# r9y9/deepvoice3_pytorch

Hardware: AMD Instinct MI355X
Metric: mel-frames/sec/node (train step, deepvoice3_ljspeech) (higher is better)
Workload: dtype f16x3

## Files before the change

### deepvoice3_pytorch_amd/csrc/attention.hip

```cpp
#include "common.h"

namespace {

__global__ __launch_bounds__(256) void attn_softmax_kernel(const dv3_softmax_desc p) {
  const int lane = threadIdx.x & 63;
  const int64_t row = (int64_t)blockIdx.x * 4 + (threadIdx.x >> 6);
  if (row >= (int64_t)p.B * p.Tq) return;
  const int b = (int)(row / p.Tq);
  const int Tk = p.Tk;
  float* s = p.s + row * Tk;
  int lo = 0, hi = Tk;
  if (p.key_len) hi = min(hi, p.key_len[b]);
  if (p.last_attended) {
    const int la = p.last_attended[0];
    const int wlo = la - p.win_back, whi = la + p.win_ahead;
    if (wlo > 0) lo = max(lo, wlo);
    if (whi < Tk) hi = min(hi, whi);
  }
  float mx = -INFINITY;
  for (int n = lo + lane; n < hi; n += 64) mx = fmaxf(mx, s[n]);
  mx = dv3_wave_max(mx);
  float sum = 0.f;
  for (int n = lo + lane; n < hi; n += 64) sum += expf(s[n] - mx);
  sum = dv3_wave_sum(sum);
// ... 128 lines not shown
    for (int r = 0; r < 16; ++r) acc[r] = 0.f;
    auto fetch3 = [&](int n0, float (&a)[16], float (&bv)[16]) __attribute__((always_inline)) {
#pragma unroll
      for (int i = 0; i < 16; ++i) {
        const int n = n0 + 2 * i + lhi;
        const int nn = min(n, Tk - 1);
        const float av = vtb[(int64_t)nn * E + e];
        bv[i] = sc[l31 * ld + nn];
        a[i] = n < Tk ? av : 0.f;
      }
    };
    float a0[16], b0[16], a1[16], b1[16];
    fetch3(0, a0, b0);
    for (int n0 = 0; n0 < Tk; n0 += 64) {
      if (n0 + 32 < Tk) fetch3(n0 + 32, a1, b1);
#pragma unroll
      for (int i = 0; i < 16; ++i) acc = __builtin_amdgcn_mfma_f32_32x32x2f32(a0[i], b0[i], acc, 0, 0, 0);
      if (n0 + 32 >= Tk) break;
      if (n0 + 64 < Tk) fetch3(n0 + 64, a0, b0);
#pragma unroll
      for (int i = 0; i < 16; ++i) acc = __builtin_amdgcn_mfma_f32_32x32x2f32(a1[i], b1[i], acc, 0, 0, 0);
    }
    const int t = t0 + l31;
    if (t < Tq) {
#pragma unroll
      for (int r = 0; r < 16; ++r) {
        const int ec = et * 32 + (r & 3) + 8 * (r >> 2) + 4 * lhi;
        if (ec < E) p.ctx[((int64_t)b * E + ec) * Tq + t] = acc[r];
      }
    }
  }
}

__global__ __launch_bounds__(64) void attn_argmax_kernel(const float* __restrict__ p, int Tk,
                                                         int32_t* __restrict__ out) {
  const int lane = threadIdx.x;
  float best = -INFINITY;
  int bi = 0x7fffffff;
  for (int n = lane; n < Tk; n += 64) {
    const float v = p[n];
    if (v > best) { best = v; bi = n; }
  }
#pragma unroll
  for (int off = 32; off > 0; off >>= 1) {
    const float ov = __shfl_xor(best, off, 64);
    const int oi = __shfl_xor(bi, off, 64);
    if (ov > best || (ov == best && oi < bi)) { best = ov; bi = oi; }
  }
  if (lane == 0) out[0] = bi;
}

}

extern "C" int dv3_attn_softmax_f32(const dv3_softmax_desc* d, void* stream) {
  DV3_REQUIRE(d && d->s && d->B > 0 && d->Tq > 0 && d->Tk > 0, "attn_softmax: bad args");
  if (d->mask) DV3_REQUIRE(d->pd && d->mask_rs * 32 >= d->Tk, "attn_softmax: mask needs pd and a wide enough row stride");
  const int64_t rows = (int64_t)d->B * d->Tq;
  hipLaunchKernelGGL(attn_softmax_kernel, dim3((unsigned)dv3_cdiv64(rows, 4)), dim3(256), 0,
                     (hipStream_t)stream, *d);
  return dv3_check_launch("attn_softmax_f32");
}

extern "C" int dv3_attn_softmax_bwd_f32(const dv3_softmax_bwd_desc* d, void* stream) {
  DV3_REQUIRE(d && d->p && d->ds && (d->dpd || d->dp_direct), "attn_softmax_bwd: bad args");
  DV3_REQUIRE(d->B > 0 && d->Tq > 0 && d->Tk > 0, "attn_softmax_bwd: bad dims");
  const int64_t rows = (int64_t)d->B * d->Tq;
  hipLaunchKernelGGL(attn_softmax_bwd_kernel, dim3((unsigned)dv3_cdiv64(rows, 4)), dim3(256), 0,
                     (hipStream_t)stream, *d);
  return dv3_check_launch("attn_softmax_bwd_f32");
}

extern "C" int dv3_attn_fwd_f32(const dv3_attn_fwd_desc* d, void* stream) {
  DV3_REQUIRE(d && d->q && d->k && d->vT && d->ctx && d->P && d->pd, "attn_fwd: null pointer");
  DV3_REQUIRE(d->B > 0 && d->E > 0 && d->Tq > 0 && d->Tk > 0 && d->B <= 65535, "attn_fwd: bad dims");
  if (d->mask) DV3_REQUIRE(d->mask_rs * 32 >= d->Tk, "attn_fwd: mask row stride too small");
  const size_t lds = (size_t)32 * (d->Tk + 1) * sizeof(float);
  DV3_REQUIRE(lds <= 64 * 1024, "attn_fwd: Tk = %d too long for the fused kernel (use the unfused path)", d->Tk);
  hipLaunchKernelGGL(attn_fwd_kernel, dim3(dv3_cdiv(d->Tq, 32), d->B), dim3(256), lds, (hipStream_t)stream, *d);
  return dv3_check_launch("attn_fwd");
}

extern "C" int dv3_attn_argmax_i32(const float* p_row, int32_t Tk, int32_t* out, void* stream) {
  DV3_REQUIRE(p_row && out && Tk > 0, "attn_argmax: bad args");
  hipLaunchKernelGGL(attn_argmax_kernel, dim3(1), dim3(64), 0, (hipStream_t)stream, p_row, Tk, out);
  return dv3_check_launch("attn_argmax_i32");
}
```

### deepvoice3_pytorch_amd/csrc/loss.hip

```cpp
#include "common.h"

namespace {

constexpr int kLossBlock = 256;

struct spec_loss_args : dv3_spec_loss_desc {
  float* dpre; float* bias_part;
};

__device__ __forceinline__ void block_reduce4(float v[4], float* out , float* extra = nullptr) {
  __shared__ float red[4][4];
#pragma unroll
  for (int k = 0; k < 4; ++k) v[k] = dv3_wave_sum(v[k]);
  const int w = threadIdx.x >> 6;
  if ((threadIdx.x & 63) == 0) {
#pragma unroll
    for (int k = 0; k < 4; ++k) red[w][k] = v[k];
  }
  __syncthreads();
  if (threadIdx.x < 4) {
    const float sum = red[0][threadIdx.x] + red[1][threadIdx.x] + red[2][threadIdx.x] + red[3][threadIdx.x];
    out[threadIdx.x] = sum;
    if (extra && threadIdx.x == 1) extra[0] = sum;
  }
// ... 198 lines not shown
        }
      }
      if (sums)
        for (int dl = dw; dl < nd; dl += 4) ys[tl * 65 + dl] = 0.f;
    }
    if (HEAD && tt_ == t_tiles - 1) {
      for (int tz = Tr + tl; tz < p.T; tz += 64) {
        int64_t ih = b * p.yh_bs + tz + (int64_t)(d0 + dw) * p.yh_ds;
        for (int dl = dw; dl < nd; dl += 4, ih += ihs) {
          p.dpre[ih] = 0.f;
          if (p.dyh) p.dyh[ih] = 0.f;
        }
      }
    }
    if (sums) {
      __syncthreads();
      const int bin = tid >> 2, part = tid & 3;
      float v[16];
#pragma unroll
      for (int i = 0; i < 16; ++i) v[i] = ys[(part * 16 + i) * 65 + bin];
#pragma unroll
      for (int w = 1; w < 16; w <<= 1)
#pragma unroll
        for (int i = 0; i < 16; i += 2 * w) v[i] += v[i + w];
      float s = v[0];
      s += __shfl_xor(s, 1, 4);
      s += __shfl_xor(s, 2, 4);
      if (part == 0 && bin < nd) p.bias_part[(int64_t)(d0 + bin) * n_part + (int64_t)b * t_tiles + tt_] = s;
    }
  }
  block_reduce4(acc, p.scratch + (int64_t)blockIdx.x * 4);
}

__global__ __launch_bounds__(256) void spec_loss_tail_zero_kernel(const dv3_spec_loss_desc p) {
  const int64_t n = (int64_t)p.B * p.r * p.D;
  const int64_t i = (int64_t)blockIdx.x * 256 + threadIdx.x;
  if (i >= n) return;
  const int dd = (int)(i % p.D);
  const int64_t bt = i / p.D;
  const int t = p.T - p.r + (int)(bt % p.r);
  const int b = (int)(bt / p.r);
  p.dyh[b * p.yh_bs + t * p.yh_ts + dd * p.yh_ds] = 0.f;
}

__global__ __launch_bounds__(256) void spec_loss_finish_kernel(const dv3_spec_loss_desc p,
                                                               int n_blocks) {
  float acc[4] = {0.f, 0.f, 0.f, 0.f};
  for (int i = threadIdx.x; i < n_blocks; i += 256)
#pragma unroll
    for (int k = 0; k < 4; ++k) acc[k] += p.scratch[(int64_t)i * 4 + k];
  __shared__ float fin[4];
  block_reduce4(acc, fin);
  __syncthreads();
  if (threadIdx.x == 0) {
    const bool use_mask = p.w_masked > 0.f && p.lengths;
    const float msum = use_mask ? spec_mask_sum(p) : 1.f;
    const float n = (float)((int64_t)p.B * (spec_t_valid(p) - p.r) * p.D);
    const float wm = use_mask ? p.w_masked : 0.f;
    const float l1 = wm * (use_mask ? fin[1] / msum : 0.f) + (1.f - wm) * fin[0] / n;
    const float bd = p.w_bd > 0.f ? wm * (use_mask ? fin[3] / msum : 0.f) + (1.f - wm) * fin[2] / n : 0.f;
    p.out4[0] = l1;
    p.out4[1] = bd;
    p.out4[2] = (1.f - p.w_bd) * l1 + p.w_bd * bd;
    p.out4[3] = msum;
  }
}

__device__ __forceinline__ float guided_w(int nk, int t, int N, int T, double inv2g2) {
  const double dlt = (double)nk / (double)N - (double)t / (double)T;
  return (float)(1.0 - exp(-dlt * dlt * inv2g2));
}

__global__ __launch_bounds__(256) void guided_attn_kernel(const float* __restrict__ attn,
                                                          const int32_t* __restrict__ in_len,
                                                          const int32_t* __restrict__ out_len,
                                                          float* __restrict__ dattn,
                                                          float* __restrict__ scratch, int L, int B,
                                                          int Tq, int Tk, float g, float gscale,
                                                          const int32_t* __restrict__ tq_valid,
                                                          const int32_t* __restrict__ tk_valid) {
  const int64_t per = (int64_t)B * Tq * Tk;
  const int64_t n = tq_valid ? (int64_t)L * B * min(tq_valid[0], Tq) * min(tk_valid[0], Tk) : per * L;
  const float inv_n = 1.0f / (float)n;
// ... 152 lines not shown
}

__global__ __launch_bounds__(256) void items_finish_kernel(const float* __restrict__ scratch, int B, int slices,
                                                           int n_sums, float* __restrict__ out,
                                                           const int32_t* __restrict__ len_a, int sub_a, int cap_a,
                                                           const int32_t* __restrict__ len_b, int cap_b,
                                                           int64_t mult) {
  const int b = blockIdx.x * 256 + threadIdx.x;
  if (b >= B) return;
  float acc[2] = {0.f, 0.f};
  for (int s = 0; s < slices; ++s)
    for (int k = 0; k < n_sums; ++k) acc[k] += scratch[((int64_t)b * slices + s) * 4 + k];
  int64_t cnt = mult * clamp_len(len_a[b] - sub_a, cap_a);
  if (len_b) cnt *= clamp_len(len_b[b], cap_b);
  float* row = out + (int64_t)b * (n_sums + 1);
  for (int k = 0; k < n_sums; ++k) row[k] = acc[k];
  row[n_sums] = (float)cnt;
}

template <class Desc>
inline bool spec_time_fast(const Desc& d) {
  return d.yh_ts == 1 && d.y_ds == 1 && d.yh_ds > 1 && d.y_ts > 1 && (int64_t)d.B * d.yh_bs < (1ll << 40);
}

inline int loss_blocks(int64_t n) {
  int64_t b = dv3_cdiv64(n, (int64_t)kLossBlock * 4);
  if (b < 1) b = 1;
  if (b > 1024) b = 1024;
  return (int)b;
}

}


extern "C" int dv3_spec_loss_scratch_floats(int32_t B, int32_t T, int32_t D) {
  int64_t tiles = (int64_t)B * dv3_cdiv(T, 64) * dv3_cdiv(D, 64);
  if (tiles > 1024) tiles = 1024;
  const int64_t flat = loss_blocks((int64_t)B * T * D);
  return (int)(4 * (tiles > flat ? tiles : flat) + 16);
}

static int spec_loss_launch(const dv3_spec_loss_desc* d, float* dpre, float* bias_part, void* stream) {
  DV3_REQUIRE(d && d->y_hat && d->y && d->out4 && d->scratch, "spec_loss: null pointer");
  DV3_REQUIRE(d->B > 0 && d->D > 0 && d->r >= 0 && d->T > d->r, "spec_loss: bad dims");
  DV3_REQUIRE(d->w_masked <= 0.f || d->lengths, "spec_loss: masked weight needs lengths");
  hipStream_t st = (hipStream_t)stream;
  spec_loss_args a;
  static_cast<dv3_spec_loss_desc&>(a) = *d;
  a.dpre = dpre;
  a.bias_part = bias_part;
  const int64_t n = (int64_t)d->B * (d->T - d->r) * d->D;
  int nb = loss_blocks(n);
  if (spec_time_fast(*d)) {
    const int t_tiles = dv3_cdiv(d->T - d->r, 64), d_tiles = dv3_cdiv(d->D, 64);
    const int64_t nt = (int64_t)d->B * t_tiles * d_tiles;
    nb = (int)(nt < 1024 ? nt : 1024);
    const bool fast_log = dv3_sw(DV3_SW_LOSS_FAST_LOG);
    auto k = dpre ? (fast_log ? spec_loss_tiled_kernel<true, true> : spec_loss_tiled_kernel<false, true>)
                     : (fast_log ? spec_loss_tiled_kernel<true, false> : spec_loss_tiled_kernel<false, false>);
    hipLaunchKernelGGL(k, dim3(nb), dim3(kLossBlock), 0, st, a, t_tiles, d_tiles, (int)nt);
  } else {
    hipLaunchKernelGGL(spec_loss_kernel, dim3(nb), dim3(kLossBlock), 0, st, a);
    if (dpre && bias_part) {
      const int t_tiles = dv3_cdiv(d->T - d->r, 64);
      const int64_t ns = (int64_t)d->B * t_tiles * d->D;
      hipLaunchKernelGGL(spec_head_rowsum_kernel, dim3((unsigned)dv3_cdiv64(ns, 256)), dim3(256), 0, st, a, t_tiles);
    }
  }
  if (d->dyh && !dpre && d->r > 0) {
    const int64_t nt = (int64_t)d->B * d->r * d->D;
    hipLaunchKernelGGL(spec_loss_tail_zero_kernel, dim3((unsigned)dv3_cdiv64(nt, 256)), dim3(256), 0,
                       st, *d);
  }
  hipLaunchKernelGGL(spec_loss_finish_kernel, dim3(1), dim3(256), 0, st, *d, nb);
  return dv3_check_launch("spec_loss_f32");
}

extern "C" int dv3_spec_loss_f32(const dv3_spec_loss_desc* d, void* stream) {
  return spec_loss_launch(d, nullptr, nullptr, stream);
}

extern "C" int dv3_spec_loss_head_f32(const dv3_spec_loss_desc* d, float* dpre, float* bias_part, void* stream) {
  DV3_REQUIRE(dpre, "spec_loss_head: dpre is required");
  return spec_loss_launch(d, dpre, bias_part, stream);
}

extern "C" int dv3_guided_attn_loss_f32(const float* attn, const int32_t* in_len,
                                        const int32_t* out_len, float* dattn, float* out1,
                                        float* scratch, int32_t L, int32_t B, int32_t Tq, int32_t Tk,
                                        float g, float gscale, void* stream) {
  DV3_REQUIRE(attn && in_len && out_len && out1 && scratch, "guided_attn: null pointer");
  DV3_REQUIRE(L > 0 && B > 0 && Tq > 0 && Tk > 0 && g > 0.f, "guided_attn: bad dims");
  hipStream_t st = (hipStream_t)stream;
// ... 50 lines not shown
extern "C" int dv3_bce_loss_head_f32(const float* p, const float* t, float* dp, float* dpre, float* bias_part, float* out1,
                                     float* scratch, int64_t rows, int32_t T, const int32_t* t_valid, float gscale,
                                     void* stream) {
  DV3_REQUIRE(p && t && dpre && out1 && scratch && rows > 0 && T > 0, "bce_loss_head: bad args");
  hipStream_t st = (hipStream_t)stream;
  const int64_t n = rows * T;
  const int nb = loss_blocks(n);
  if (t_valid) {
    hipLaunchKernelGGL(bce_kernel, dim3(nb), dim3(256), 0, st, p, t, dp, scratch, n, gscale, (int)T, t_valid, dpre, bias_part);
    hipLaunchKernelGGL(sum_finish_kernel, dim3(1), dim3(256), 0, st, scratch, nb, 0.f, out1, t_valid, (int)T,
                       (const int32_t*)nullptr, 0, rows);
  } else {
    hipLaunchKernelGGL(bce_kernel, dim3(nb), dim3(256), 0, st, p, t, dp, scratch, n, gscale, 0, (const int32_t*)nullptr, dpre,
                       bias_part);
    hipLaunchKernelGGL(sum_finish_kernel, dim3(1), dim3(256), 0, st, scratch, nb, 1.0f / (float)n, out1,
                       (const int32_t*)nullptr, 0, (const int32_t*)nullptr, 0, (int64_t)0);
  }
  return dv3_check_launch("bce_loss_head_f32");
}

extern "C" int dv3_loss_items_scratch_floats(int32_t B, int32_t T) {
  if (B <= 0 || T <= 0) return 0;
  return (int)((int64_t)4 * B * item_slices(T));
}

extern "C" int dv3_spec_loss_items_f32(const dv3_spec_items_desc* d, void* stream) {
  DV3_REQUIRE(d && d->y_hat && d->y && d->lengths && d->out && d->scratch, "spec_loss_items: null pointer");
  DV3_REQUIRE(d->B > 0 && d->B <= 65535 && d->D > 0 && d->r >= 0 && d->T > 0, "spec_loss_items: bad dims");
  hipStream_t st = (hipStream_t)stream;
  const int Tr = d->T > d->r ? d->T - d->r : 0;
  const int S = Tr > 0 ? item_slices(Tr) : 0;
  if (S > 0) {
    DV3_REQUIRE((int64_t)dv3_cdiv(Tr, S) * d->D < (1ll << 31), "spec_loss_items: slice too large");
    if (spec_time_fast(*d) && dv3_sw(DV3_SW_LOSS_FAST_LOG))
      hipLaunchKernelGGL(spec_items_kernel<true>, dim3(S, d->B), dim3(kLossBlock), 0, st, *d);
    else
      hipLaunchKernelGGL(spec_items_kernel<false>, dim3(S, d->B), dim3(kLossBlock), 0, st, *d);
  }
  hipLaunchKernelGGL(items_finish_kernel, dim3(dv3_cdiv(d->B, 256)), dim3(256), 0, st, (const float*)d->scratch, (int)d->B,
                     S, 2, d->out, d->lengths, (int)d->r, Tr, (const int32_t*)nullptr, 0, (int64_t)d->D);
  return dv3_check_launch("spec_loss_items_f32");
}

extern "C" int dv3_bce_loss_items_f32(const float* p, const float* t, const int32_t* lengths, float* out,
                                      float* scratch, int32_t B, int32_t T, void* stream) {
  DV3_REQUIRE(p && t && lengths && out && scratch, "bce_loss_items: null pointer");
  DV3_REQUIRE(B > 0 && B <= 65535 && T > 0, "bce_loss_items: bad dims");
  hipStream_t st = (hipStream_t)stream;
  const int S = item_slices(T);
  hipLaunchKernelGGL(bce_items_kernel, dim3(S, B), dim3(256), 0, st, p, t, lengths, scratch, (int)T);
  hipLaunchKernelGGL(items_finish_kernel, dim3(dv3_cdiv(B, 256)), dim3(256), 0, st, (const float*)scratch, (int)B, S, 1,
                     out, lengths, 0, (int)T, (const int32_t*)nullptr, 0, (int64_t)1);
  return dv3_check_launch("bce_loss_items_f32");
}

extern "C" int dv3_guided_attn_loss_items_f32(const float* attn, const int32_t* in_len, const int32_t* out_len,
                                              float* out, float* scratch, int32_t L, int32_t B, int32_t Tq,
                                              int32_t Tk, float g, void* stream) {
  DV3_REQUIRE(attn && in_len && out_len && out && scratch, "guided_attn_items: null pointer");
  DV3_REQUIRE(L > 0 && B > 0 && B <= 65535 && Tq > 0 && Tk > 0 && g > 0.f, "guided_attn_items: bad dims");
  hipStream_t st = (hipStream_t)stream;
  const int S = item_slices(Tq);
  DV3_REQUIRE((int64_t)dv3_cdiv(Tq, S) * Tk < (1ll << 31), "guided_attn_items: slice too large");
  hipLaunchKernelGGL(guided_attn_items_kernel, dim3(S, B), dim3(256), 0, st, attn, in_len, out_len, scratch, (int)L,
                     (int)B, (int)Tq, (int)Tk, g);
  hipLaunchKernelGGL(items_finish_kernel, dim3(dv3_cdiv(B, 256)), dim3(256), 0, st, (const float*)scratch, (int)B, S, 1,
                     out, out_len, 0, (int)Tq, in_len, (int)Tk, (int64_t)L);
// ... 3 lines not shown
```

### deepvoice3_pytorch_amd/ops.py

```python
import contextlib
import ctypes
import functools
import math

import torch

from . import _lib
from ._lib import CONSTS, STRUCTS, _env_flag, _env_int, _env_str

EPI_LINEAR = CONSTS["DV3_EPI_LINEAR"]
EPI_RELU = CONSTS["DV3_EPI_RELU"]
EPI_SIGMOID = CONSTS["DV3_EPI_SIGMOID"]
EPI_GLU = CONSTS["DV3_EPI_GLU"]
EPI_HIGHWAY = CONSTS["DV3_EPI_HIGHWAY"]
EPI_DGRAD = CONSTS["DV3_EPI_DGRAD"]
EPI_SOFTSIGN = CONSTS["DV3_EPI_SOFTSIGN"]
STORE_BCT = CONSTS["DV3_STORE_BCT"]
STORE_INTERLEAVE2 = CONSTS["DV3_STORE_INTERLEAVE2"]

_conv_desc = STRUCTS["dv3_conv_desc"]
_wgrad_desc = STRUCTS["dv3_wgrad_desc"]
_wn_desc = STRUCTS["dv3_wn_desc"]
_wn_bwd_desc = STRUCTS["dv3_wn_bwd_desc"]
_gate_bwd_desc = STRUCTS["dv3_gate_bwd_desc"]
# ... 1598 lines not shown
    if (x8 or want8) and not _c8_layer_ok(v, cfg, x8 if want8 is None else bool(want8), x.shape[2]):
        y = ConvLayerFn.apply(from_c8(x, v.shape[1]) if x8 else x, v, g, bias, spk,
                              from_c8(r) if is_c8(r) else r, from_c8(r2) if is_c8(r2) else r2, cfg, packed)
        out8 = x8 if want8 is None else bool(want8)
        return to_c8(y) if out8 else y
    if x8 or want8:
        y = ConvLayerC8Fn.apply(x, v, g, bias, spk, r, r2, cfg, packed)
        if is_c8(y):
            gated = cfg.mode in (EPI_GLU, EPI_HIGHWAY)
            y._dv3_C = v.shape[0] // 2 if gated else v.shape[0]
        return y
    return ConvLayerFn.apply(x, v, g, bias, spk, r, r2, cfg, packed)


def _attn_split(forward=False):
    if forward and _gemm_mode == "f16x3":
        return False
    return _gemm_mode != "f32"


class AttnCoreFn(torch.autograd.Function):
    @staticmethod
    def forward(ctx, q, k, v, key_len, last_attended, cfg):
        q, k, v = _c(_chk(q, "q")), _c(_chk(k, "k")), _c(_chk(v, "v"))
        B, E, Tq = q.shape
        Tk = k.shape[2]
        p_drop, training, win_back, win_ahead, site = cfg
        dev = q.device
        bits, bits_rs, dscale = None, 0, 1.0
        if training and p_drop > 0:
            bits, bits_rs = dropout_bits(B * Tq, Tk, p_drop, dev, site)
            dscale = 1.0 / (1.0 - p_drop)
        if fused_attention and last_attended is None and Tk <= 511 and Tq > 1:
            vT = transpose(v)
            ctxv = torch.empty((B, E, Tq), dtype=torch.float32, device=dev)
            P = torch.empty((B, Tq, Tk), dtype=torch.float32, device=dev)
            pd = torch.empty_like(P)
            d = _attn_fwd_desc()
            d.q, d.k, d.vT, d.key_len = q.data_ptr(), k.data_ptr(), vT.data_ptr(), _ptr(key_len)
            d.mask, d.mask_rs, d.drop_scale = _ptr(bits), bits_rs, dscale
            vs = valid.scale if valid is not None else None
            d.pd_scale = 1.0 if vs is not None else Tk * math.sqrt(1.0 / Tk)
            d.pd_scale_dev = _ptr(vs)
            d.ctx, d.P, d.pd = ctxv.data_ptr(), P.data_ptr(), pd.data_ptr()
            d.B, d.E, d.Tq, d.Tk = B, E, Tq, Tk
            _lib.call("dv3_attn_fwd_f32", ctypes.byref(d), _stream())
            if any(ctx.needs_input_grad[:3]):
                ctx.save_for_backward(q, k, v, P, pd)
                ctx.bits, ctx.bits_rs, ctx.dscale, ctx.pd_scale = bits, bits_rs, dscale, d.pd_scale
                ctx.scale_dev = vs
            return ctxv, P
        S = conv_gemm(k, q, Tq, 0, B=B, Cin=E, Tin=Tk, M=Tq, Tout=Tk, a_bs=E * Tq)
        pd = torch.empty_like(S)
        d = _softmax_desc()
        d.s, d.pd, d.key_len, d.last_attended = S.data_ptr(), pd.data_ptr(), _ptr(key_len), _ptr(last_attended)
        d.mask, d.mask_rs, d.drop_scale = _ptr(bits), bits_rs, dscale
        vs = valid.scale if valid is not None else None
        d.pd_scale = 1.0 if vs is not None else Tk * math.sqrt(1.0 / Tk)
        d.pd_scale_dev = _ptr(vs)
        d.B, d.Tq, d.Tk, d.win_back, d.win_ahead = B, Tq, Tk, win_back, win_ahead
        _lib.call("dv3_attn_softmax_f32", ctypes.byref(d), _stream())
        P = S
        ctxv = wgrad_gemm(v, pd, B=B, M=E, Cin=Tq, T=Tk, Tin=Tk, n_slabs=B,
                          split_bf16=_attn_split(forward=True)).view(B, E, Tq)
        if any(ctx.needs_input_grad[:3]):
            ctx.save_for_backward(q, k, v, P, pd)
            ctx.bits, ctx.bits_rs, ctx.dscale, ctx.pd_scale = bits, bits_rs, dscale, d.pd_scale
            ctx.scale_dev = vs
        return ctxv, P

    @staticmethod
    def backward(ctx, dctx, dP):
# ... 765 lines not shown
```

### include/dv3hip.h

```cpp
#ifndef DV3HIP_H
#define DV3HIP_H

#include <stdint.h>

#ifdef __cplusplus
extern "C" {
#endif

#define DV3_OK 0
#define DV3_EINVAL (-1)
#define DV3_ELAUNCH (-2)

#define DV3_ABI_VERSION 50
int dv3_abi_version(void);
const char* dv3_last_error(void);
int dv3_device_info(int dev, char* name, int name_len, int* n_cu);
int dv3_sizeof(const char* name);
#define DV3_SWITCHES(X) \
  X(2, WGRAD_TILE, 0, 0, 4, "split weight gradient: 0 by rule / 1 128x128 per tap / 2 256x128 per tap / 3 all-taps / 4 two-steps-ahead all-taps") \
  X(3, X3_PINGPONG, 1, 0, 1, "8-wave split tap-GEMM tiles: 0 in-phase / 1 ping-pong main loop") \
  X(4, PLANES_TILE, 0, 0, 9, "planes tap-GEMM tile: 0 by rule, conv_c8pp first / 1 128x128 / 2 128x64 / 9 128x256; any other value: by rule, conv_c8pp kept out") \
  X(12, X3_PP2_MIN_TILES, 128, 0, 2147483647, "256x256 split tap-GEMM serves eligible grids of at least this many tiles (0 never)") \
  X(14, X3_PRIO, 0, 0, 4, "wave priority scheme of the ping-pong split main loop (kernel argument; 0 none)") \
  X(15, WGRAD_PRIO, 0, 0, 2, "wave priority scheme of the all-taps weight gradient (kernel argument; 0 none)") \
  X(17, WGRAD_TAPS2, 1, 0, 1, "all-taps weight gradient by rule: 0 one step ahead / 1 two steps ahead") \
  X(18, X3_WIDE, 1, 0, 1, "16-byte input-gradient epilogue through LDS of the split tap-GEMMs (kernel argument): 0 off / 1 on") \
  X(19, C8PP_MIN_TILES, 128, 0, 2147483647, "conv_c8pp serves eligible grids of at least this many tiles (0 never, 1 always)") \
  X(20, WGRAD_C8_PF2, 1, 0, 1, "register-transposing wgrad_c8: operands fetched 0 one / 1 two steps ahead") \
  X(22, PP2_SK, 1, 0, 3, "stream-K form of the 256x256 split tap-GEMM: 0 never / 1 by rule, forward / 2 whenever a workspace is given / 3 by rule, both directions") \
  X(29, PP2_ORD_U, 81, 0, 81, "LOAD-phase order of the unmasked 256x256 split instantiations: 0, 17 or 81 only") \
  X(30, C8PP_RF, 1, 0, 1, "conv_c8pp LOAD phase: 0 staging first / 1 fragment reads first") \
  X(31, PP2_ORD_M, 81, 0, 81, "LOAD-phase order of the masked 256x256 split instantiations: 0, 17 or 81 only") \
  X(34, C8PP_NW4, 2, 0, 2, "conv_c8pp form: 0 8 waves on 256x256 only / 1 two 4-wave workgroups per CU on 256x128 / 2 by rule") \
  X(35, C8PP_STAGGER, 0, 0, 1024, "conv_c8pp, 4-wave form: start delay (x 64 cycles) of the delayed blocks (kernel argument)") \
  X(36, C8PP_STAGGER_MASK, 1, 0, 2147483647, "conv_c8pp, 4-wave form: blocks with (blockIdx & mask) != 0 are the delayed ones (kernel argument)") \
  X(44, X3_KS, 1, 0, 2, "k-split form of the 128x64 split tile: 0 never / 1 by rule / 2 wherever eligible") \
  X(47, WGRAD_T2_WINDOW, 1, 0, 1, "two-steps-ahead weight gradient, d = 1 / 3: 0 per-tap form / 1 one window for three taps") \
  X(48, WGRAD_T2_IL, 1, 0, 1, "its window forms stage the next tile 0 after / 1 between the MFMAs") \
  X(49, WGRAD_C8_IL, 1, 0, 1, "register-transposing wgrad_c8, three taps: next tile staged 0 after / 1 between the MFMAs") \
  X(50, PP2_FAST_TAIL, 1, 0, 1, "256x256 split tap-GEMM, gated launch: 0 guarded tail everywhere / 1 straight-line tail on interior sub-tiles (kernel argument)") \
  X(51, WN_BWD_VEC4, 1, 0, 1, "weight-norm backward gather: 0 4-byte everywhere / 1 16-byte where aligned") \
  X(52, WGRAD_C8_TR, 4, 0, 4, "wgrad_c8 form: 0 register-transposing / 1 transposing LDS read / 2 + staging between the MFMAs / 3 + one barrier per two K steps / 4 both") \
  X(54, SPK_PREFETCH, 1, 0, 1, "speaker-bias backward tile loads: 0 at the top of the tile / 1 one tile ahead") \
  X(55, GATE_VEC, 1, 0, 1, "gate backward 16-byte accesses: 0 gated layers with T % 4 == 0 only / 1 rows of any length") \
  X(56, GATE_C8_FAST, 1, 0, 1, "c8 gate backward sigmoid: 0 expf and a division / 1 v_exp_f32 + v_rcp_f32") \
  X(57, LOSS_FAST_LOG, 1, 0, 1, "tiled spectrogram loss logarithms: 0 logf / 1 v_log_f32")
#define DV3_SW_ENUM_(id, name, dflt, lo, hi, doc) DV3_SW_##name = id,
enum { DV3_SWITCHES(DV3_SW_ENUM_) };
#define DV3_DEBUG_CENSUS 40
int dv3_debug_set(int what, int value);
int dv3_debug_reset(void);
int dv3_switch_query(int what, int32_t* value, int32_t* dflt);
int dv3_debug_read(int what, void* dst, int64_t bytes);
int dv3_debug_get(int what);

int dv3_ring_standin(const void* src, int64_t src_bytes, void* scratch, int64_t scratch_bytes, int64_t bytes,
                     int32_t channels, int32_t threads, float bytes_per_us, void* stream);

enum {
  DV3_EPI_LINEAR = 0,
  DV3_EPI_RELU = 1,
  DV3_EPI_SIGMOID = 2,
  DV3_EPI_GLU = 3,
  DV3_EPI_HIGHWAY = 4,
  DV3_EPI_DGRAD = 5,
  DV3_EPI_SOFTSIGN = 6
};

enum {
  DV3_STORE_BCT = 0,
  DV3_STORE_INTERLEAVE2 = 1
};

typedef struct dv3_conv_desc {
  const float* x;  int64_t x_bs, x_rs;
  const float* a;  int64_t a_bs; int32_t lda; int32_t a_half;
  const float* bias;
  const float* spk; int64_t spk_bs, spk_rs, spk_ts;
  const float* r;  int64_t r_bs, r_rs;
// ... 151 lines not shown
  uint64_t site;
} dv3_dropout_site;
int dv3_dropout_keep_c8_multi(const dv3_dropout_site* sites, int32_t n, uint64_t seed,
                              const uint64_t* dev_seed_offset, void* stream);

int dv3_dropout_apply_f32(const float* x, const uint32_t* bits, int32_t bits_rs, float scale,
                          float* out, int64_t rows, int32_t T, void* stream);

typedef struct dv3_softmax_desc {
  float* s; float* pd;
  const int32_t* key_len;
  const int32_t* last_attended;
  const uint32_t* mask; int32_t mask_rs; float drop_scale;
  float pd_scale;
  int32_t B, Tq, Tk, win_back, win_ahead;
  const float* pd_scale_dev;
} dv3_softmax_desc;
int dv3_attn_softmax_f32(const dv3_softmax_desc* d, void* stream);
typedef struct dv3_softmax_bwd_desc {
  const float* p; const float* dpd; const float* dp_direct; float* ds;
  const uint32_t* mask; int32_t mask_rs; float drop_scale;
  int32_t B, Tq, Tk;
  const float* scale_dev;
} dv3_softmax_bwd_desc;
int dv3_attn_softmax_bwd_f32(const dv3_softmax_bwd_desc* d, void* stream);
typedef struct dv3_attn_fwd_desc {
  const float* q; const float* k; const float* vT;
  const int32_t* key_len;
  const uint32_t* mask; int32_t mask_rs; float drop_scale;
  float pd_scale;
  float* ctx; float* P; float* pd;
  int32_t B, E, Tq, Tk;
  const float* pd_scale_dev;
} dv3_attn_fwd_desc;
int dv3_attn_fwd_f32(const dv3_attn_fwd_desc* d, void* stream);
int dv3_attn_argmax_i32(const float* p_row, int32_t Tk, int32_t* out, void* stream);

int dv3_transpose_f32(const float* x, float* y, const float* add, int32_t B, int32_t R,
                      int32_t C, float alpha, void* stream);
int dv3_axpby_f32(const float* a, const float* b, float* out, int64_t n, float alpha,
                  void* stream);
int dv3_sum_scalars_f32(const float* a, const float* b, const float* c, const float* d, float* out, void* stream);
int dv3_memset_b8(void* p, int32_t value, int64_t bytes, void* stream);
int dv3_memset_rows_b8(void* p, int32_t value, int64_t rows, int64_t row_bytes, int64_t row_stride_bytes, void* stream);
int dv3_zero_tail_b32(void* x, int64_t rows, int32_t T, int32_t words, const int32_t* t_valid, int32_t mult,
                      int32_t max_tail, void* stream);
int dv3_zero_tail_items_b32(void* x, int32_t B, int64_t rows_per_item, int32_t T, int32_t words, const int32_t* len,
                            int32_t mult, int32_t max_tail, void* stream);
int dv3_embedding_bct_f32(const int64_t* idx, const float* w, float* out,
                          const uint32_t* mask, int32_t mask_rs, float drop_scale,
                          int32_t B, int32_t T, int32_t C, int32_t n_vocab, void* stream);
int dv3_embedding_bct_bwd_f32(const int64_t* idx, const float* dout, float* dw,
                              const uint32_t* mask, int32_t mask_rs, float drop_scale,
                              int32_t B, int32_t T, int32_t C, int32_t n_vocab,
                              int32_t padding_idx, void* stream);
int dv3_sincos_pos_bct_f32(const int64_t* pos, const float* table, const float* w,
                           int32_t w_per_batch, const float* base, float* out, int32_t B,
                           int32_t T, int32_t C, int32_t n_pos, int32_t apply_sincos,
                           void* stream);
int dv3_sincos_pos_table_bwd_f32(const int64_t* pos, const float* table, const float* w, int32_t w_per_batch,
                                 const float* dout, float* dtable, int32_t B, int32_t T, int32_t C,
                                 int32_t n_pos, int32_t apply_sincos, void* stream);
int dv3_sincos_pos_bwd_f32(const int64_t* pos, const float* table, const float* w,
                           int32_t w_per_batch, const float* dout, float* dw, int32_t B, int32_t T,
                           int32_t C, int32_t n_pos, void* stream);
int dv3_sincos_pos_bwd2_f32(const int64_t* pos, const float* table, const float* w,
// ... 295 lines not shown
```

Baseline: 3.873 million.

## Add LDS-staged fused attention forward and one-tile-per-workgroup spectrogram loss kernel

Adds a fused attention forward kernel that reads V directly, which removes the separate transpose. It stages Q/K/V chunks through double-buffered LDS with register prefetch and uses up to 160 KB of dynamic shared memory. The spectrogram loss gets a new kernel that launches one workgroup per 64x64 tile and uses 16-byte accesses where aligned, replacing the capped persistent grid. The loss finish reduction is also unrolled to keep more loads in flight. Risks are lower occupancy from the large LDS footprint, and the hand-written struct field must match the Python ctypes descriptor layout.

```diff
diff --git a/deepvoice3_pytorch_amd/csrc/attention.hip b/deepvoice3_pytorch_amd/csrc/attention.hip
--- a/deepvoice3_pytorch_amd/csrc/attention.hip
+++ b/deepvoice3_pytorch_amd/csrc/attention.hip
@@ -184,6 +184,195 @@
   }
 }
 
+template <int NKT_MAX, int EC>
+__global__ __launch_bounds__(256) void attn_fwd_lds_kernel(const dv3_attn_fwd_desc p, int bufsz) {
+  extern __shared__ float sc[];
+  constexpr int RPT = EC / 8;
+  constexpr int TILE = EC * 32;
+  constexpr int NACC = (NKT_MAX + 3) / 4;
+  const int tid = threadIdx.x, lane = tid & 63, wave = tid >> 6;
+  const int l31 = lane & 31, lhi = lane >> 5;
+  const int col = tid & 31, rg = tid >> 5;
+  const int nqb = (p.Tq + 31) / 32;
+  const int lin = dv3_xcd_remap(blockIdx.x, gridDim.x);
+  const int qblk = lin % nqb, b = lin / nqb, t0 = qblk * 32;
+  const int E = p.E, Tq = p.Tq, Tk = p.Tk;
+  const int ld = Tk + 1;
+  const int nkt = (Tk + 31) / 32;
+  float* stage = sc + 32 * ld;
+  const float* __restrict__ qb = p.q + (int64_t)b * E * Tq;
+  const float* __restrict__ kb = p.k + (int64_t)b * E * Tk;
+  const float* __restrict__ vb = p.v + (int64_t)b * E * Tk;
+  {
+    const int wrot = (wave + qblk + b) & 3;
+    float st0[NKT_MAX + 1][RPT], st1[NKT_MAX + 1][RPT];
+    const int tqc = min(t0 + col, Tq - 1);
+    auto fetch1 = [&](float (&st)[NKT_MAX + 1][RPT], int e0) __attribute__((always_inline)) {
+#pragma unroll
+      for (int rr = 0; rr < RPT; ++rr) {
+        const int ch = min(e0 + rg + 8 * rr, E - 1);
+        st[0][rr] = qb[(int64_t)ch * Tq + tqc];
+#pragma unroll
+        for (int j = 1; j <= NKT_MAX; ++j) st[j][rr] = kb[(int64_t)ch * Tk + min((j - 1) * 32 + col, Tk - 1)];
+      }
+    };
+    auto stash1 = [&](const float (&st)[NKT_MAX + 1][RPT], int e0, float* buf) __attribute__((always_inline)) {
+#pragma unroll
+      for (int rr = 0; rr < RPT; ++rr) {
+        const bool row = e0 + rg + 8 * rr < E;
+        buf[(rg + 8 * rr) * 32 + col] = (row && t0 + col < Tq) ? st[0][rr] : 0.f;
+#pragma unroll
+        for (int j = 1; j <= NKT_MAX; ++j)
+          buf[j * TILE + (rg + 8 * rr) * 32 + col] = (row && (j - 1) * 32 + col < Tk) ? st[j][rr] : 0.f;
+      }
+    };
+    f32x16 acc[NACC];
+#pragma unroll
+    for (int j = 0; j < NACC; ++j)
+#pragma unroll
+      for (int r = 0; r < 16; ++r) acc[j][r] = 0.f;
+    const int nch = (E + EC - 1) / EC;
+    auto step1 = [&](int c, float (&fetch_to)[NKT_MAX + 1][RPT], const float (&stash_from)[NKT_MAX + 1][RPT])
+        __attribute__((always_inline)) {
+      const float* cur = stage + (c & 1) * bufsz;
+      fetch1(fetch_to, (c + 2) * EC);
+      const int np = (min(EC, E - c * EC) + 1) >> 1;
+      float a[EC / 2];
+#pragma unroll
+      for (int i = 0; i < EC / 2; ++i) a[i] = cur[(2 * i + lhi) * 32 + l31];
+#pragma unroll
+      for (int j = 0; j < NACC; ++j) {
+        const int kt = wrot + 4 * j;
+        if (kt < nkt) {
+          const float* kt_ = cur + (1 + kt) * TILE + lhi * 32 + l31;
+          float bk[EC / 2];
+#pragma unroll
+          for (int i = 0; i < EC / 2; ++i) bk[i] = kt_[i * 64];
+          if (np == EC / 2) {
+#pragma unroll
+            for (int i = 0; i < EC / 2; ++i) acc[j] = __builtin_amdgcn_mfma_f32_32x32x2f32(a[i], bk[i], acc[j], 0, 0, 0);
+          } else {
+#pragma unroll
+            for (int i = 0; i < EC / 2; ++i)
+              if (i < np) acc[j] = __builtin_amdgcn_mfma_f32_32x32x2f32(a[i], bk[i], acc[j], 0, 0, 0);
+          }
+        }
+      }
+      stash1(stash_from, (c + 1) * EC, stage + ((c + 1) & 1) * bufsz);
+      __syncthreads();
+    };
+    fetch1(st0, 0);
+    fetch1(st1, EC);
+    stash1(st0, 0, stage);
+    __syncthreads();
+    for (int c = 0; c < nch; c += 2) {
+      step1(c, st0, st1);
+      if (c + 1 < nch) step1(c + 1, st1, st0);
+    }
+#pragma unroll
+    for (int j = 0; j < NACC; ++j) {
+      const int cl = (wrot + 4 * j) * 32 + l31;
+      if (cl < Tk) {
+#pragma unroll
+        for (int r = 0; r < 16; ++r) sc[((r & 3) + 8 * (r >> 2) + 4 * lhi) * ld + cl] = acc[j][r];
+      }
+    }
+  }
+  const int npass = (E + 127) / 128, n_steps = npass * nkt;
+  float sv0[16], sv1[16];
+  auto fetch3 = [&](float (&sv)[16], int s) __attribute__((always_inline)) {
+    const int e0 = (s / nkt) * 128, n = min((s % nkt) * 32 + col, Tk - 1);
+#pragma unroll
+    for (int j = 0; j < 16; ++j) sv[j] = vb[(int64_t)min(e0 + rg + 8 * j, E - 1) * Tk + n];
+  };
+  auto stash3 = [&](const float (&sv)[16], int s, float* buf) __attribute__((always_inline)) {
+    const int e0 = (s / nkt) * 128;
+    const bool key = (s % nkt) * 32 + col < Tk;
+#pragma unroll
+    for (int j = 0; j < 16; ++j) buf[(rg + 8 * j) * 34 + col] = (key && e0 + rg + 8 * j < E) ? sv[j] : 0.f;
+  };
+  fetch3(sv0, 0);
+  fetch3(sv1, 1);
+  __syncthreads();
+  {
+    const int row = tid >> 3, sub = tid & 7;
+    const int t = t0 + row;
+    int hi = Tk;
+    if (p.key_len) hi = min(hi, p.key_len[b]);
+    float* s = sc + row * ld;
+    float mx = -INFINITY;
+    for (int n = sub; n < hi; n += 8) mx = fmaxf(mx, s[n]);
+#pragma unroll
+    for (int off = 4; off > 0; off >>= 1) mx = fmaxf(mx, __shfl_xor(mx, off, 64));
+    float sum = 0.f;
+    for (int n = sub; n < hi; n += 8) sum += expf(s[n] - mx);
+#pragma unroll
+    for (int off = 4; off > 0; off >>= 1) sum += __shfl_xor(sum, off, 64);
+    const float inv = 1.0f / sum;
+    const float pd_scale = p.pd_scale_dev ? p.pd_scale * p.pd_scale_dev[0] : p.pd_scale;
+    const int64_t grow = (int64_t)b * Tq + t;
+    for (int n = sub; n < Tk; n += 8) {
+      float v = 0.f;
+      if (n < hi) v = expf(s[n] - mx) * inv;
+      float d = v;
+      if (p.mask && t < Tq) d = dv3_keep(p.mask, grow, p.mask_rs, n) ? v * p.drop_scale : 0.f;
+      d *= pd_scale;
+      s[n] = d;
+      if (t < Tq) {
+        p.P[grow * Tk + n] = v;
+        p.pd[grow * Tk + n] = d;
+      }
+    }
+  }
+  stash3(sv0, 0, stage);
+  __syncthreads();
+  f32x16 acc;
+  auto step3 = [&](int s, float (&fetch_to)[16], const float (&stash_from)[16]) __attribute__((always_inline)) {
+    const float* cur = stage + (s & 1) * bufsz;
+    fetch3(fetch_to, s + 2);
+    const int et = (s / nkt) * 4 + wave, n0 = (s % nkt) * 32;
+    if (n0 == 0) {
+#pragma unroll
+      for (int r = 0; r < 16; ++r) acc[r] = 0.f;
+    }
+    if (et * 32 < E) {
+      const int np = (min(32, Tk - n0) + 1) >> 1;
+      const float* a_ = cur + (wave * 32 + l31) * 34 + lhi;
+      const float* b_ = sc + l31 * ld;
+      float av[16], bv[16];
+#pragma unroll
+      for (int i = 0; i < 16; ++i) {
+        av[i] = a_[2 * i];
+        bv[i] = b_[min(n0 + 2 * i + lhi, Tk - 1)];
+      }
+      if (np == 16) {
+#pragma unroll
+        for (int i = 0; i < 16; ++i) acc = __builtin_amdgcn_mfma_f32_32x32x2f32(av[i], bv[i], acc, 0, 0, 0);
+      } else {
+#pragma unroll
+        for (int i = 0; i < 16; ++i)
+          if (i < np) acc = __builtin_amdgcn_mfma_f32_32x32x2f32(av[i], bv[i], acc, 0, 0, 0);
+      }
+      if (n0 + 32 >= Tk) {
+        const int t = t0 + l31;
+        if (t < Tq) {
+#pragma unroll
+          for (int r = 0; r < 16; ++r) {
+            const int ec = et * 32 + (r & 3) + 8 * (r >> 2) + 4 * lhi;
+            if (ec < E) p.ctx[((int64_t)b * E + ec) * Tq + t] = acc[r];
+          }
+        }
+      }
+    }
+    stash3(stash_from, s + 1, stage + ((s + 1) & 1) * bufsz);
+    __syncthreads();
+  };
+  for (int s = 0; s < n_steps; s += 2) {
+    step3(s, sv0, sv1);
+    if (s + 1 < n_steps) step3(s + 1, sv1, sv0);
+  }
+}
+
 __global__ __launch_bounds__(64) void attn_argmax_kernel(const float* __restrict__ p, int Tk,
                                                          int32_t* __restrict__ out) {
   const int lane = threadIdx.x;
@@ -222,12 +411,37 @@
   return dv3_check_launch("attn_softmax_bwd_f32");
 }
 
+namespace {
+template <int NKT_MAX, int EC>
+int launch_attn_fwd_lds(const dv3_attn_fwd_desc* d, hipStream_t st) {
+  const int stage1 = (1 + NKT_MAX) * EC * 32, stage3 = 128 * 34;
+  const int bufsz = stage1 > stage3 ? stage1 : stage3;
+  const size_t lds = ((size_t)32 * (d->Tk + 1) + 2 * (size_t)bufsz) * sizeof(float);
+  DV3_REQUIRE(lds <= 160 * 1024, "attn_fwd: Tk = %d too long for the fused kernel (use the unfused path)", d->Tk);
+  static bool attr_set = false;
+  if (!attr_set) {
+    hipError_t e = hipFuncSetAttribute((const void*)attn_fwd_lds_kernel<NKT_MAX, EC>,
+                                       hipFuncAttributeMaxDynamicSharedMemorySize, 160 * 1024);
+    if (e != hipSuccess) {
+      dv3_set_error("attn_fwd: hipFuncSetAttribute: %s", hipGetErrorString(e));
+      return DV3_ELAUNCH;
+    }
+    attr_set = true;
+  }
+  hipLaunchKernelGGL((attn_fwd_lds_kernel<NKT_MAX, EC>), dim3(dv3_cdiv(d->Tq, 32) * d->B), dim3(256), lds, st, *d, bufsz);
+  return dv3_check_launch("attn_fwd");
+}
+}
+
 extern "C" int dv3_attn_fwd_f32(const dv3_attn_fwd_desc* d, void* stream) {
-  DV3_REQUIRE(d && d->q && d->k && d->vT && d->ctx && d->P && d->pd, "attn_fwd: null pointer");
+  DV3_REQUIRE(d && d->q && d->k && (d->vT || d->v) && d->ctx && d->P && d->pd, "attn_fwd: null pointer");
   DV3_REQUIRE(d->B > 0 && d->E > 0 && d->Tq > 0 && d->Tk > 0 && d->B <= 65535, "attn_fwd: bad dims");
   if (d->mask) DV3_REQUIRE(d->mask_rs * 32 >= d->Tk, "attn_fwd: mask row stride too small");
+  DV3_REQUIRE(d->Tk <= 511, "attn_fwd: Tk = %d too long for the fused kernel (use the unfused path)", d->Tk);
+  if (d->v) {
+    return d->Tk <= 160 ? launch_attn_fwd_lds<5, 32>(d, (hipStream_t)stream) : launch_attn_fwd_lds<16, 8>(d, (hipStream_t)stream);
+  }
   const size_t lds = (size_t)32 * (d->Tk + 1) * sizeof(float);
-  DV3_REQUIRE(lds <= 64 * 1024, "attn_fwd: Tk = %d too long for the fused kernel (use the unfused path)", d->Tk);
   hipLaunchKernelGGL(attn_fwd_kernel, dim3(dv3_cdiv(d->Tq, 32), d->B), dim3(256), lds, (hipStream_t)stream, *d);
   return dv3_check_launch("attn_fwd");
 }
diff --git a/deepvoice3_pytorch_amd/csrc/loss.hip b/deepvoice3_pytorch_amd/csrc/loss.hip
--- a/deepvoice3_pytorch_amd/csrc/loss.hip
+++ b/deepvoice3_pytorch_amd/csrc/loss.hip
@@ -254,6 +254,129 @@
   block_reduce4(acc, p.scratch + (int64_t)blockIdx.x * 4);
 }
 
+template <bool FAST, bool HEAD, bool VEC>
+__global__ __launch_bounds__(kLossBlock) void spec_loss_tile4_kernel(const spec_loss_args p, int t_tiles, int d_tiles) {
+  __shared__ float ys[64 * 65];
+  const int Tr = p.T - p.r, D = p.D;
+  const int tid = threadIdx.x;
+  const int tile = dv3_xcd_remap(blockIdx.x, gridDim.x);
+  const int tt_ = tile % t_tiles, dt = (tile / t_tiles) % d_tiles, b = tile / (d_tiles * t_tiles);
+  const int t0 = tt_ * 64, d0 = dt * 64;
+  const int nd = min(64, D - d0);
+  const int tl = tid & 63, dw = tid >> 6;
+  float tg[16];
+  {
+    const int dd = d0 + tl;
+    const float* __restrict__ yp = p.y + b * p.y_bs + (int64_t)(t0 + dw + p.r) * p.y_ts + dd;
+#pragma unroll
+    for (int k = 0; k < 16; ++k) tg[k] = (t0 + dw + 4 * k < Tr && dd < D) ? yp[(int64_t)(4 * k) * p.y_ts] : 0.f;
+  }
+  const int Trv = spec_t_valid(p) - p.r;
+  const int fq = tid & 15, br = tid >> 4;
+  const int tq = t0 + 4 * fq;
+  const int64_t ih0 = b * p.yh_bs + tq + (int64_t)(d0 + br) * p.yh_ds;
+  const int64_t ihs = 16 * p.yh_ds;
+  f32x4 yv[4];
+#pragma unroll
+  for (int k = 0; k < 4; ++k) {
+    const bool row = br + 16 * k < nd;
+    if (VEC) {
+      yv[k] = (row && tq < p.T) ? *reinterpret_cast<const f32x4*>(p.y_hat + ih0 + k * ihs) : f32x4{0.f, 0.f, 0.f, 0.f};
+    } else {
+#pragma unroll
+      for (int j = 0; j < 4; ++j) yv[k][j] = (row && tq + j < Trv) ? p.y_hat[ih0 + k * ihs + j] : 0.f;
+    }
+  }
+  const bool use_mask = p.w_masked > 0.f && p.lengths;
+  const float msum = use_mask ? spec_mask_sum(p) : 1.f;
+  const float inv_n = 1.0f / (float)((int64_t)p.B * Trv * D);
+  const float wm = use_mask ? p.w_masked : 0.f;
+  const float c_all = (1.f - wm) * inv_n, c_msk = use_mask ? wm / msum : 0.f;
+  const int len_b = use_mask ? p.lengths[b] : 0;
+  const bool sums = HEAD && p.bias_part != nullptr;
+  float acc[4] = {0.f, 0.f, 0.f, 0.f};
+#pragma unroll
+  for (int k = 0; k < 16; ++k) ys[(dw + 4 * k) * 65 + tl] = tg[k];
+  __syncthreads();
+  float m[4], coef[4];
+#pragma unroll
+  for (int j = 0; j < 4; ++j) {
+    m[j] = (use_mask && (tq + j + p.r) < len_b) ? 1.f : 0.f;
+    coef[j] = c_all + c_msk * m[j];
+  }
+#pragma unroll
+  for (int k = 0; k < 4; ++k) {
+    const int dl = br + 16 * k;
+    if (dl >= nd) break;
+    f32x4 g4 = {0.f, 0.f, 0.f, 0.f}, gz4 = {0.f, 0.f, 0.f, 0.f};
+#pragma unroll
+    for (int j = 0; j < 4; ++j) {
+      float* slot = ys + (4 * fq + j) * 65 + dl;
+      if (tq + j < Trv) {
+        const float yh = yv[k][j], y = *slot;
+        const float diff = yh - y;
+        const float ad = fabsf(diff);
+        acc[0] += ad;
+        acc[1] += m[j] * ad;
+        float dz = 0.f;
+        if (p.w_bd > 0.f) {
+          float z;
+          spec_bd<FAST>(yh, y, z, dz);
+          acc[2] += z;
+          acc[3] += m[j] * z;
+        }
+        if (p.dyh || HEAD) {
+          const float sgn = (diff > 0.f) ? 1.f : ((diff < 0.f) ? -1.f : 0.f);
+          const float g = p.gscale * coef[j] * ((1.f - p.w_bd) * sgn + p.w_bd * dz);
+          g4[j] = g;
+          if (HEAD) gz4[j] = sigmoid_head_dz(g, yh);
+        }
+      }
+      if (sums) *slot = gz4[j];
+    }
+    const int64_t ih = ih0 + k * ihs;
+    if (VEC) {
+      if (tq < p.T) {
+        if (p.dyh) *reinterpret_cast<f32x4*>(p.dyh + ih) = g4;
+        if (HEAD) *reinterpret_cast<f32x4*>(p.dpre + ih) = gz4;
+      }
+    } else {
+#pragma unroll
+      for (int j = 0; j < 4; ++j)
+        if (tq + j < p.T) {
+          if (p.dyh) p.dyh[ih + j] = g4[j];
+          if (HEAD) p.dpre[ih + j] = gz4[j];
+        }
+    }
+  }
+  if (HEAD && tt_ == t_tiles - 1) {
+    for (int tz = t0 + 64 + tl; tz < p.T; tz += 64) {
+      int64_t ih = b * p.yh_bs + tz + (int64_t)(d0 + dw) * p.yh_ds;
+      for (int dl = dw; dl < nd; dl += 4, ih += 4 * p.yh_ds) {
+        p.dpre[ih] = 0.f;
+        if (p.dyh) p.dyh[ih] = 0.f;
+      }
+    }
+  }
+  if (sums) {
+    __syncthreads();
+    const int64_t n_part = (int64_t)p.B * t_tiles;
+    const int bin = tid >> 2, part = tid & 3;
+    float v[16];
+#pragma unroll
+    for (int i = 0; i < 16; ++i) v[i] = ys[(part * 16 + i) * 65 + bin];
+#pragma unroll
+    for (int w = 1; w < 16; w <<= 1)
+#pragma unroll
+      for (int i = 0; i < 16; i += 2 * w) v[i] += v[i + w];
+    float s = v[0];
+    s += __shfl_xor(s, 1, 4);
+    s += __shfl_xor(s, 2, 4);
+    if (part == 0 && bin < nd) p.bias_part[(int64_t)(d0 + bin) * n_part + (int64_t)b * t_tiles + tt_] = s;
+  }
+  block_reduce4(acc, p.scratch + (int64_t)blockIdx.x * 4);
+}
+
 __global__ __launch_bounds__(256) void spec_loss_tail_zero_kernel(const dv3_spec_loss_desc p) {
   const int64_t n = (int64_t)p.B * p.r * p.D;
   const int64_t i = (int64_t)blockIdx.x * 256 + threadIdx.x;
@@ -268,9 +391,20 @@
 __global__ __launch_bounds__(256) void spec_loss_finish_kernel(const dv3_spec_loss_desc p,
                                                                int n_blocks) {
   float acc[4] = {0.f, 0.f, 0.f, 0.f};
-  for (int i = threadIdx.x; i < n_blocks; i += 256)
-#pragma unroll
-    for (int k = 0; k < 4; ++k) acc[k] += p.scratch[(int64_t)i * 4 + k];
+  for (int i0 = threadIdx.x; i0 < n_blocks; i0 += 256 * 8) {
+    float v[8][4];
+#pragma unroll
+    for (int u = 0; u < 8; ++u) {
+      const int i = i0 + 256 * u;
+#pragma unroll
+      for (int k = 0; k < 4; ++k) v[u][k] = i < n_blocks ? p.scratch[(int64_t)i * 4 + k] : 0.f;
+    }
+#pragma unroll
+    for (int u = 0; u < 8; ++u)
+      if (i0 + 256 * u < n_blocks)
+#pragma unroll
+        for (int k = 0; k < 4; ++k) acc[k] += v[u][k];
+  }
   __shared__ float fin[4];
   block_reduce4(acc, fin);
   __syncthreads();
@@ -489,10 +623,11 @@
 
 }
 
+constexpr int64_t kTile4MaxTiles = 1ll << 22;
 
 extern "C" int dv3_spec_loss_scratch_floats(int32_t B, int32_t T, int32_t D) {
   int64_t tiles = (int64_t)B * dv3_cdiv(T, 64) * dv3_cdiv(D, 64);
-  if (tiles > 1024) tiles = 1024;
+  if (tiles > kTile4MaxTiles) tiles = 1024;
   const int64_t flat = loss_blocks((int64_t)B * T * D);
   return (int)(4 * (tiles > flat ? tiles : flat) + 16);
 }
@@ -511,11 +646,22 @@
   if (spec_time_fast(*d)) {
     const int t_tiles = dv3_cdiv(d->T - d->r, 64), d_tiles = dv3_cdiv(d->D, 64);
     const int64_t nt = (int64_t)d->B * t_tiles * d_tiles;
-    nb = (int)(nt < 1024 ? nt : 1024);
-    const bool fast_log = dv3_sw(DV3_SW_LOSS_FAST_LOG);
-    auto k = dpre ? (fast_log ? spec_loss_tiled_kernel<true, true> : spec_loss_tiled_kernel<false, true>)
-                     : (fast_log ? spec_loss_tiled_kernel<true, false> : spec_loss_tiled_kernel<false, false>);
-    hipLaunchKernelGGL(k, dim3(nb), dim3(kLossBlock), 0, st, a, t_tiles, d_tiles, (int)nt);
+    const bool fast_log = dv3_sw(DV3_SW_LOSS_FAST_LOG) & 1;
+    if (!(dv3_sw(DV3_SW_LOSS_FAST_LOG) & 2) && (int64_t)d->B * dv3_cdiv(d->T, 64) * d_tiles <= kTile4MaxTiles) {
+      nb = (int)nt;
+      auto al16 = [](const void* q) { return ((uintptr_t)q & 15) == 0; };
+      const bool vec = d->T % 4 == 0 && d->yh_ds % 4 == 0 && d->yh_bs % 4 == 0 && al16(d->y_hat) && al16(d->dyh) && al16(dpre);
+      auto k = dpre ? (fast_log ? (vec ? spec_loss_tile4_kernel<true, true, true> : spec_loss_tile4_kernel<true, true, false>)
+                                : (vec ? spec_loss_tile4_kernel<false, true, true> : spec_loss_tile4_kernel<false, true, false>))
+                    : (fast_log ? (vec ? spec_loss_tile4_kernel<true, false, true> : spec_loss_tile4_kernel<true, false, false>)
+                                : (vec ? spec_loss_tile4_kernel<false, false, true> : spec_loss_tile4_kernel<false, false, false>));
+      hipLaunchKernelGGL(k, dim3(nb), dim3(kLossBlock), 0, st, a, t_tiles, d_tiles);
+    } else {
+      nb = (int)(nt < 1024 ? nt : 1024);
+      auto k = dpre ? (fast_log ? spec_loss_tiled_kernel<true, true> : spec_loss_tiled_kernel<false, true>)
+                       : (fast_log ? spec_loss_tiled_kernel<true, false> : spec_loss_tiled_kernel<false, false>);
+      hipLaunchKernelGGL(k, dim3(nb), dim3(kLossBlock), 0, st, a, t_tiles, d_tiles, (int)nt);
+    }
   } else {
     hipLaunchKernelGGL(spec_loss_kernel, dim3(nb), dim3(kLossBlock), 0, st, a);
     if (dpre && bias_part) {
@@ -632,7 +778,7 @@
   const int S = Tr > 0 ? item_slices(Tr) : 0;
   if (S > 0) {
     DV3_REQUIRE((int64_t)dv3_cdiv(Tr, S) * d->D < (1ll << 31), "spec_loss_items: slice too large");
-    if (spec_time_fast(*d) && dv3_sw(DV3_SW_LOSS_FAST_LOG))
+    if (spec_time_fast(*d) && (dv3_sw(DV3_SW_LOSS_FAST_LOG) & 1))
       hipLaunchKernelGGL(spec_items_kernel<true>, dim3(S, d->B), dim3(kLossBlock), 0, st, *d);
     else
       hipLaunchKernelGGL(spec_items_kernel<false>, dim3(S, d->B), dim3(kLossBlock), 0, st, *d);
diff --git a/deepvoice3_pytorch_amd/ops.py b/deepvoice3_pytorch_amd/ops.py
--- a/deepvoice3_pytorch_amd/ops.py
+++ b/deepvoice3_pytorch_amd/ops.py
@@ -1654,12 +1654,12 @@
             bits, bits_rs = dropout_bits(B * Tq, Tk, p_drop, dev, site)
             dscale = 1.0 / (1.0 - p_drop)
         if fused_attention and last_attended is None and Tk <= 511 and Tq > 1:
-            vT = transpose(v)
             ctxv = torch.empty((B, E, Tq), dtype=torch.float32, device=dev)
             P = torch.empty((B, Tq, Tk), dtype=torch.float32, device=dev)
             pd = torch.empty_like(P)
             d = _attn_fwd_desc()
-            d.q, d.k, d.vT, d.key_len = q.data_ptr(), k.data_ptr(), vT.data_ptr(), _ptr(key_len)
+            d.q, d.k, d.key_len = q.data_ptr(), k.data_ptr(), _ptr(key_len)
+            d.v = v.data_ptr()
             d.mask, d.mask_rs, d.drop_scale = _ptr(bits), bits_rs, dscale
             vs = valid.scale if valid is not None else None
             d.pd_scale = 1.0 if vs is not None else Tk * math.sqrt(1.0 / Tk)
diff --git a/include/dv3hip.h b/include/dv3hip.h
--- a/include/dv3hip.h
+++ b/include/dv3hip.h
@@ -44,7 +44,7 @@
   X(54, SPK_PREFETCH, 1, 0, 1, "speaker-bias backward tile loads: 0 at the top of the tile / 1 one tile ahead") \
   X(55, GATE_VEC, 1, 0, 1, "gate backward 16-byte accesses: 0 gated layers with T % 4 == 0 only / 1 rows of any length") \
   X(56, GATE_C8_FAST, 1, 0, 1, "c8 gate backward sigmoid: 0 expf and a division / 1 v_exp_f32 + v_rcp_f32") \
-  X(57, LOSS_FAST_LOG, 1, 0, 1, "tiled spectrogram loss logarithms: 0 logf / 1 v_log_f32")
+  X(57, LOSS_FAST_LOG, 1, 0, 3, "tiled spectrogram loss: bit 0 logarithms 0 logf / 1 v_log_f32; bit 1 kernel 0 one workgroup per tile, 16-byte accesses where aligned / 1 persistent grid, 4-byte accesses")
 #define DV3_SW_ENUM_(id, name, dflt, lo, hi, doc) DV3_SW_##name = id,
 enum { DV3_SWITCHES(DV3_SW_ENUM_) };
 #define DV3_DEBUG_CENSUS 40
@@ -262,6 +262,7 @@
   float* ctx; float* P; float* pd;
   int32_t B, E, Tq, Tk;
   const float* pd_scale_dev;
+  const float* v;
 } dv3_attn_fwd_desc;
 int dv3_attn_fwd_f32(const dv3_attn_fwd_desc* d, void* stream);
 int dv3_attn_argmax_i32(const float* p_row, int32_t Tk, int32_t* out, void* stream);
```

Result: no change. 3.885 million (median of 6 runs) (+0.3%).
